# krzkro4122/vit-gan

Hardware: AMD Instinct MI355X
Metric: images/sec (G+D step) ViTGAN 32x32 patch4 dim384 (higher is better)
Workload: dtype bf16; 1 GPU; C2: CIFAR-10-shaped 3x32x32, patch 4 (65 tokens), E=384, 4 heads, 6 blocks ViT discriminator + SLN/SIREN generator (z=1024, 32 tokens, 4 blocks), full alternating G+D step, AdamW; fp8_attention=False, per_gpu_batch=256, global_batch=256, loss=ns, parallelism=dp1, hip_graph=True, compress_mapping_grad=False, fused_real_fake_pass=True, losses_finite=True

## Files before the change

include/vitgan_hip.h:

```cpp
#ifndef VITGAN_HIP_H
#define VITGAN_HIP_H

#include <stdint.h>

#ifdef __cplusplus
extern "C" {
#endif

#define VG_ABI_VERSION 9
int vg_abi_version(void);


int vg_linear_fwd(const void* A, const void* W, const float* bias, const void* res, void* C,
                  void* pre_bf16, float* pre_f32, int M, int N, int K, int act, float act_scale,
                  void* stream);
int vg_linear_gelu_fwd(const void* A, const void* W, const float* bias, void* C, void* dcode, int M, int N, int K,
                       void* stream);
int vg_linear_dgrad(const void* dY, const void* W, void* dX, int M, int N, int K, int mul_mode,
                    const void* Z, const float* Zf, float act_scale, void* stream);
#define VG_WGRAD_MAX_SPLITS 64
long long vg_linear_wgrad_slab_floats(int N, int K, int splits);
int vg_linear_wgrad(const void* dY, const void* X, float* dW, float* slab_ws, long long slab_floats, int M,
                    int N, int K, int splits, int accumulate, void* stream);
int vg_linear_wgrad_group(int n, const void* const* dY, const void* const* X, const int* N, const int* K, const long long* off,
// ... 49 lines not shown

long long vg_encoder_post_attention_image_elems(void);
int vg_encoder_post_attention_pack(const void* Wo, const void* W1, const void* W2, void* img, void* stream);
int vg_encoder_post_attention_fwd(const void* ao, const void* x, const void* img, const float* bo, const float* b1, const float* b2,
                                  const float* gamma2, const float* beta2, const float* gamma, const float* beta, void* xmid, void* xn2,
                                  float* mean2, float* rstd2, void* a1, void* dcode, void* Y, void* Yn, float* mean, float* rstd, int M,
                                  float eps, float drop_p, unsigned long long seed, int site_attn, int site_mlp,
                                  const unsigned* step_dev, void* stream);

int vg_linear_sln_fwd(const void* A, const void* Wp, const float* bias, const void* res, const float* resf, int res_period,
                      void* Y, void* Yn, float* mean, float* rstd, const void* wmod, const float* lw, const float* lb,
                      const float* gs, const float* bs, int M, int K, float eps, float drop_p, unsigned long long seed,
                      int site, const unsigned* step_dev, void* stream);
int vg_linear_dgrad_sln_bwd(const void* dY, const void* WpT, const void* h, int h_bcast_rows, const void* wmod,
                            const float* mean, const float* rstd, const float* lw, const float* lb, const float* gs,
                            const float* bs, const void* gres, void* dh, void* dhm, float* dw_acc, int dw_accumulate,
                            float* part, int M, int K, float drop_p, unsigned long long seed, int site,
                            const unsigned* step_dev, void* stream);

int vg_colsum_f32(const float* part, int rows, int width, float* d0, int n0, float* d1, int n1,
                  float* d2, int n2, float* d3, int n3, int accumulate, void* stream);

int vg_colsum_bf16_parts(int R);
int vg_colsum_bf16(const void* X, long long ld, int R, int N, float* part_ws, float* dst, int accumulate,
                   void* stream);

int vg_dropout_apply(const void* x, void* y, long long n, float p, unsigned long long seed, int site,
                     const unsigned* step_dev, void* stream);

int vg_attention_fwd(const void* qkv, void* out, float* lse, int B, int H, int S, int HE,
                     float scale, void* stream);
int vg_attention_bwd(const void* qkv, const void* out, const void* d_out, const float* lse,
                     void* d_qkv, int B, int H, int S, int HE, float scale, void* stream);
int vg_attention_cls_fwd(const void* qkv, void* out_cls, float* lse_cls, int B, int H, int S, int HE, float scale, void* stream);
int vg_attention_cls_bwd(const void* qkv, const void* out_cls, const void* d_out_cls, const float* lse_cls, void* d_qkv, int B, int H,
                         int S, int HE, float scale, void* stream);

int vg_attention_fp8_fwd(const void* qkv, void* out, float* lse, int B, int H, int S, int HE,
                         float scale, void* stream);
int vg_attention_fp8_bwd(const void* qkv, const void* out, const void* d_out, const float* lse,
                         void* d_qkv, int B, int H, int S, int HE, float scale, void* stream);

int vg_attention_l2_fwd(const void* qkv, void* out, float* lse, int B, int H, int S, int HE,
                        float scale, void* stream);
int vg_attention_l2_bwd(const void* qkv, const void* out, const void* d_out, const float* lse,
                        void* d_qkv, int B, int H, int S, int HE, float scale, void* stream);

int vg_unfold_tokens_fwd(const void* img, int img_is_bf16, void* tokens, int B, int C, int IH, int P,
                         int overlap, void* stream);
int vg_unfold_tokens_bwd(const void* d_tokens, void* d_img, int B, int C, int IH, int P, int overlap,
                         void* stream);

int vg_act_fwd(const void* h, void* y, long long n, int act, void* stream);
int vg_act_bwd(const void* dy, const void* h, void* dh, long long n, int act, void* stream);
int vg_act_bwd_bwd(const void* u, const void* dy, const void* h, void* d_dy, void* d_h, long long n, int act,
                   void* stream);
int vg_layernorm_bwd_bwd_parts(int R);
int vg_layernorm_bwd_bwd(const void* u, const void* dy, const void* x, const float* mean, const float* rstd,
                         const float* gamma, void* d_dy, void* d_x, float* part, int R, int E, void* stream);
int vg_attention_bwd_bwd(const void* qkv, const void* d_out, const float* lse, const void* u_qkv, void* d_d_out,
                         void* d_qkv2, int B, int H, int S, int HE, float scale, void* stream);

int vg_zero_tick(float* g, long long n, int* step_dev, void* stream);
int vg_step_inputs(const float* real, void* imgs_bf16, long long n_img, float* z, long long n_z,
                   unsigned long long seed, const int* step_dev, void* stream);

// ... 199 lines not shown
```

vit-gan_amd/_lib.py:

```python
from __future__ import annotations

import ctypes as C
import os
import subprocess
from typing import Optional

_HERE = os.path.dirname(os.path.abspath(__file__))
LIB_PATH = os.environ.get("VITGAN_HIP_LIB", os.path.join(_HERE, "libvitgan_hip.so"))
CSRC = os.path.join(_HERE, "csrc")

c_void_p, c_int, c_float, c_ll = C.c_void_p, C.c_int, C.c_float, C.c_longlong
ABI_VERSION = 9


class VgVitDims(C.Structure):
    _fields_ = [(n, c_int) for n in ("C", "IH", "P", "E", "H", "L", "R", "Kc")]


class VgVitLayout(C.Structure):
    _fields_ = [(n, c_ll) for n in (
        "conv_w", "conv_b", "pos", "cls", "layer0", "layer_stride", "wqkv", "wo", "w1", "w2",
        "ln1_w", "ln1_b", "bqkv", "bo", "ln2_w", "ln2_b", "b1", "b2", "layer_weights",
        "lnf_w", "lnf_b", "hw1", "hb1", "hw2", "hb2", "total")]

# ... 53 lines not shown
    "vg_linear_wgrad_slab_floats": (c_ll, [c_int, c_int, c_int]),
    "vg_linear_wgrad": (c_int, [P, P, P, P, c_ll, c_int, c_int, c_int, c_int, c_int, P]),
    "vg_linear_wgrad_group": (c_int, [c_int, P, P, P, P, P, c_int, c_int, P, c_ll, P, c_ll, c_int, P]),
    "vg_layernorm_fwd": (c_int, [P, c_ll, P, P, P, c_ll, P, P, c_int, c_int, c_float, P]),
    "vg_layernorm_bwd_parts": (c_int, [c_int]),
    "vg_layernorm_bwd": (c_int, [P, P, P, P, P, P, P, P, c_int, c_int, P]),
    "vg_sln_fwd": (c_int, [P, c_int, P, P, P, P, P, P, P, P, c_int, c_int, c_float, P]),
    "vg_sln_bwd": (c_int, [P, P, c_int, P, P, P, P, P, P, P, P, P, P, c_int, P, c_int, c_int, P]),
    "vg_row_pack_elems": (c_ll, [c_int]),
    "vg_row_pack_weight": (c_int, [P, c_int, c_int, c_int, P, P]),
    "vg_row_parts": (c_int, [c_int]),
    "vg_linear_ln_fwd": (c_int, [P, P, P, P, P, P, P, P, P, P, c_int, c_int, c_float, c_float, C.c_ulonglong, c_int, P, P]),
    "vg_linear_dgrad_ln_bwd": (c_int, [P, P, P, P, P, P, P, P, P, P, c_int, c_int, c_float, C.c_ulonglong, c_int, P, P]),
    "vg_row_pack_elems_e": (c_ll, [c_int, c_int]),
    "vg_row_pack_weight_e": (c_int, [c_int, P, c_int, c_int, c_int, P, P]),
    "vg_linear_ln_fwd_e": (c_int, [c_int, P, P, P, P, P, P, P, P, P, P, c_int, c_int, c_float, c_float, C.c_ulonglong, c_int, P, P]),
    "vg_linear_dgrad_ln_bwd_e": (c_int, [c_int, P, P, P, P, P, P, P, P, P, P, c_int, c_int, c_float, C.c_ulonglong, c_int, P, P]),
    "vg_linear_sln_fwd_e": (c_int, [c_int, P, P, P, P, P, c_int, P, P, P, P, P, P, P, P, P, c_int, c_int, c_float, c_float, C.c_ulonglong, c_int, P, P]),
    "vg_linear_dgrad_sln_bwd_e": (c_int, [c_int, P, P, P, c_int, P, P, P, P, P, P, P, P, P, P, P, c_int, P, c_int, c_int, c_float, C.c_ulonglong, c_int, P, P]),
    "vg_encoder_mlp_image_elems": (c_ll, []),
    "vg_encoder_mlp_pack": (c_int, [P, P, P, P]),
    "vg_encoder_mlp_fwd": (c_int, [P, P, P, P, P, P, P, P, P, P, P, P, P, c_int, c_float, c_float, C.c_ulonglong, c_int, P, P]),
    "vg_encoder_post_attention_image_elems": (c_ll, []),
    "vg_encoder_post_attention_pack": (c_int, [P, P, P, P, P]),
    "vg_encoder_post_attention_fwd": (c_int, [P] * 20 + [c_int, c_float, c_float, C.c_ulonglong, c_int, c_int, P, P]),
    "vg_linear_sln_fwd": (c_int, [P, P, P, P, P, c_int, P, P, P, P, P, P, P, P, P, c_int, c_int, c_float, c_float, C.c_ulonglong, c_int, P, P]),
    "vg_linear_dgrad_sln_bwd": (c_int, [P, P, P, c_int, P, P, P, P, P, P, P, P, P, P, P, c_int, P, c_int, c_int, c_float, C.c_ulonglong, c_int, P, P]),
    "vg_colsum_f32": (c_int, [P, c_int, c_int, P, c_int, P, c_int, P, c_int, P, c_int, c_int, P]),
    "vg_colsum_bf16_parts": (c_int, [c_int]),
    "vg_colsum_bf16": (c_int, [P, c_ll, c_int, c_int, P, P, c_int, P]),
    "vg_dropout_apply": (c_int, [P, P, c_ll, c_float, C.c_ulonglong, c_int, P, P]),
    "vg_attention_fwd": (c_int, [P, P, P, c_int, c_int, c_int, c_int, c_float, P]),
    "vg_attention_bwd": (c_int, [P, P, P, P, P, c_int, c_int, c_int, c_int, c_float, P]),
    "vg_attention_cls_fwd": (c_int, [P, P, P, c_int, c_int, c_int, c_int, c_float, P]),
    "vg_attention_cls_bwd": (c_int, [P, P, P, P, P, c_int, c_int, c_int, c_int, c_float, P]),
    "vg_unfold_tokens_fwd": (c_int, [P, c_int, P, c_int, c_int, c_int, c_int, c_int, P]),
    "vg_unfold_tokens_bwd": (c_int, [P, P, c_int, c_int, c_int, c_int, c_int, P]),
    "vg_attention_fp8_fwd": (c_int, [P, P, P, c_int, c_int, c_int, c_int, c_float, P]),
    "vg_attention_fp8_bwd": (c_int, [P, P, P, P, P, c_int, c_int, c_int, c_int, c_float, P]),
    "vg_attention_l2_fwd": (c_int, [P, P, P, c_int, c_int, c_int, c_int, c_float, P]),
    "vg_attention_l2_bwd": (c_int, [P, P, P, P, P, c_int, c_int, c_int, c_int, c_float, P]),
    "vg_act_fwd": (c_int, [P, P, c_ll, c_int, P]),
    "vg_act_bwd": (c_int, [P, P, P, c_ll, c_int, P]),
    "vg_act_bwd_bwd": (c_int, [P, P, P, P, P, c_ll, c_int, P]),
    "vg_layernorm_bwd_bwd_parts": (c_int, [c_int]),
    "vg_layernorm_bwd_bwd": (c_int, [P, P, P, P, P, P, P, P, P, c_int, c_int, P]),
    "vg_attention_bwd_bwd": (c_int, [P, P, P, P, P, P, c_int, c_int, c_int, c_int, c_float, P]),
    "vg_zero_tick": (c_int, [P, c_ll, P, P]),
    "vg_step_inputs": (c_int, [P, P, c_ll, P, c_ll, C.c_ulonglong, P, P]),
    "vg_diffaug_fwd": (c_int, [P, P, P, c_int, c_int, c_int, c_int, C.c_ulonglong, c_int, P, P]),
    "vg_diffaug_bwd": (c_int, [P, P, c_int, c_int, c_int, c_int, c_int, C.c_ulonglong, c_int, P, P]),
    "vg_diffaug_p_fwd": (c_int, [P, P, P, c_int, c_int, c_int, c_int, C.c_ulonglong, c_int, P, P, P]),
    "vg_diffaug_p_bwd": (c_int, [P, P, c_int, c_int, c_int, c_int, c_int, C.c_ulonglong, c_int, P, P, P]),
    "vg_ada_update": (c_int, [P, c_int, P, c_float, c_float, c_int, P, P]),
    "vg_gan_loss": (c_int, [P, P, P, c_int, c_int, c_int, c_float, P]),
    "vg_gan_loss_pair": (c_int, [P, P, P, c_int, c_int, c_int, c_int, c_int, c_float, P]),
    "vg_bcr_loss": (c_int, [P, P, P, P, P, c_int, c_int, c_int, c_float, c_float, c_int, c_int, c_float, P]),
    "vg_adamw_step": (c_int, [P, P, P, P, P, c_ll, c_float, c_float, c_float, c_float, c_float, c_int, P, c_float, P]),
    "vg_adamw_ema_step": (c_int, [P, P, P, P, P, P, c_ll, c_float, c_float, c_float, c_float, c_float, c_int, P, c_float, c_float, c_int, P]),
    "vg_adamw_step_dlr": (c_int, [P, P, P, P, P, c_ll, P, c_float, c_float, c_float, c_float, c_int, P, c_float, P]),
    "vg_adamw_ema_step_dlr": (c_int, [P, P, P, P, P, P, c_ll, P, c_float, c_float, c_float, c_float, c_int, P, c_float, c_float, c_int, P]),
    "vg_lr_schedule": (c_int, [C.POINTER(VgLrSched), C.POINTER(VgLrSched), P, P, P, P]),
    "vg_ema_update": (c_int, [P, P, c_ll, c_float, c_int, c_int, P, P]),
    "vg_diversity_loss": (c_int, [P, P, P, P, c_int, c_int, c_float, P]),
    "vg_grad_clip": (c_int, [P, c_ll, c_float, c_float, P, P]),
    "vg_cast_f32_bf16": (c_int, [P, P, c_ll, P]),
# ... 94 lines not shown
```

vit-gan_amd/csrc/attention.hip:

```cpp
#include "vg_attn.h"
#include "vg_kernels.h"

typedef long fp8x8;
__device__ __forceinline__ fp8x8 to_fp8(float a0, float a1, float a2, float a3, float a4, float a5, float a6, float a7) {
  int lo = 0, hi = 0;
  lo = __builtin_amdgcn_cvt_pk_fp8_f32(a0, a1, lo, false);
  lo = __builtin_amdgcn_cvt_pk_fp8_f32(a2, a3, lo, true);
  hi = __builtin_amdgcn_cvt_pk_fp8_f32(a4, a5, hi, false);
  hi = __builtin_amdgcn_cvt_pk_fp8_f32(a6, a7, hi, true);
  return (fp8x8)(((unsigned long)(unsigned)hi << 32) | (unsigned long)(unsigned)lo);
}
__device__ __forceinline__ fp8x8 to_fp8(bf16x8 v) {
  return to_fp8(vg_bf2f(v[0]), vg_bf2f(v[1]), vg_bf2f(v[2]), vg_bf2f(v[3]), vg_bf2f(v[4]), vg_bf2f(v[5]), vg_bf2f(v[6]), vg_bf2f(v[7]));
}
__device__ __forceinline__ fp8x8 pack_pair_fp8(f32x4 a, f32x4 b, float mul) {
  return to_fp8(a[0] * mul, a[1] * mul, a[2] * mul, a[3] * mul, b[0] * mul, b[1] * mul, b[2] * mul, b[3] * mul);
}
__device__ __forceinline__ f32x4 vg_mfma_fp8(fp8x8 a, fp8x8 b, f32x4 c) { return __builtin_amdgcn_mfma_f32_16x16x32_fp8_fp8(a, b, c, 0, 0, 0); }
template <bool FP8>
__device__ __forceinline__ f32x4 score_mfma(bf16x8 a, bf16x8 b, f32x4 c) {
  if constexpr (FP8) return vg_mfma_fp8(to_fp8(a), to_fp8(b), c);
  else return vg_mfma(a, b, c);
}
#define VG_P_FP8_SCALE 256.0f
// ... 383 lines not shown
      f32x4 s = zero, dp = zero;
#pragma unroll
      for (int ks = 0; ks < KS; ++ks) {
        s = score_mfma<FP8>(lfrag_row<HE>(s0, 16 * qt, ks, lane), kf[ks], s);
        dp = vg_mfma(lfrag_row<HE>(s1, 16 * qt, ks, lane), vf[ks], dp);
      }
      const f32x4 lq4 = *(const f32x4*)(ll + 16 * qt + 4 * g);
      const f32x4 dl4 = *(const f32x4*)(dl + 16 * qt + 4 * g);
#pragma unroll
      for (int r = 0; r < 4; ++r) {
        const int q = 16 * qt + 4 * g + r;
        const float p = ((q < S) && (key < S)) ? __expf(s[r] * scale - lq4[r]) : 0.f;
        pr[qt][r] = p;
        ds[qt][r] = p * (dp[r] - dl4[r]) * scale;
      }
    }
    bf16x8 pf[KP], dsf[KP];
#pragma unroll
    for (int u = 0; u < KP; ++u) {
      const int hi = (2 * u + 1 < NT) ? 2 * u + 1 : 0;
      pf[u] = pack_pair(pr[2 * u], (2 * u + 1 < NT) ? pr[hi] : zero);
      dsf[u] = pack_pair(ds[2 * u], (2 * u + 1 < NT) ? ds[hi] : zero);
    }
    bf16* rowp = dqb + (size_t)(key < S ? key : 0) * ld;
#pragma unroll
    for (int pp = 0; pp < DT / 2; ++pp) {
      f32x4 dv[2] = {zero, zero}, dk[2] = {zero, zero};
#pragma unroll
      for (int u = 0; u < KP; ++u) {
#pragma unroll
        for (int t = 0; t < 2; ++t) {
          dv[t] = vg_mfma(lfrag_tr<HE>(s1, u, 32 * pp + 16 * t, lane), pf[u], dv[t]);
          dk[t] = vg_mfma(lfrag_tr<HE>(s0, u, 32 * pp + 16 * t, lane), dsf[u], dk[t]);
        }
      }
      store_tiles<2>(rowp + E + 32 * pp, dk, 1.0f, g, key < S);
      store_tiles<2>(rowp + 2 * E + 32 * pp, dv, 1.0f, g, key < S);
    }
  }
}

template <int HE>
__global__ __launch_bounds__(320, 2) void vg_attn_bwd_bwd2_kernel(const bf16* __restrict__ qkv, const bf16* __restrict__ d_o,
                                                                  const float* __restrict__ lse, const bf16* __restrict__ uqkv,
                                                                  bf16* __restrict__ d_do, bf16* __restrict__ d_qkv, int B, int S, int H,
                                                                  float scale, const void* __restrict__ zeros) {
  constexpr int NT = 5, KS = HE / 32, DT = HE / 16, KP = 3, RP = 96;
  constexpr int IMG = RP * HE * 2;
  __shared__ __attribute__((aligned(16))) unsigned char sm[4 * IMG + 4 * RP * 4];
  unsigned char* i0 = sm;
  unsigned char* i1 = sm + IMG;
  unsigned char* i2 = sm + 2 * IMG;
  unsigned char* i3 = sm + 3 * IMG;
  float* dl = (float*)(sm + 4 * IMG);
  float* gm = dl + RP;
  float* pl = gm + RP;
  float* ll = pl + RP;
  int b, h;
  if (!attn_block(B, H, b, h)) return;
  const int tid = threadIdx.x, lane = tid & 63, wv = tid >> 6;
  const int g = lane >> 4, li = lane & 15;
  const int E = H * HE;
  const size_t ld = 3 * (size_t)E;
  const bf16* qb = qkv + (size_t)b * S * ld + h * HE;
  const bf16* kb = qb + E;
  const bf16* vb = qb + 2 * E;
// ... 160 lines not shown
    for (int pp = 0; pp < DT / 2; ++pp) {
      f32x4 dk[2] = {zero, zero}, dv[2] = {zero, zero};
#pragma unroll
      for (int u = 0; u < KP; ++u)
#pragma unroll
        for (int t = 0; t < 2; ++t) {
          const int d0 = 32 * pp + 16 * t;
          dk[t] = vg_mfma(lfrag_tr<HE>(i2, u, d0, lane), dsf[u], dk[t]);
          dk[t] = vg_mfma(lfrag_tr<HE>(i0, u, d0, lane), sgf[u], dk[t]);
          dv[t] = vg_mfma(lfrag_tr<HE>(i1, u, d0, lane), hf[u], dv[t]);
        }
      store_tiles<2>(rowp + E + 32 * pp, dk, scale, g, key < S);
      store_tiles<2>(rowp + 2 * E + 32 * pp, dv, 1.0f, g, key < S);
    }
  }
}

__device__ __attribute__((aligned(16))) unsigned int vg_attn_zero_page[4] = {0u, 0u, 0u, 0u};
static const void* attn_zeros() {
  static void* zp = nullptr;
  if (!zp && hipGetSymbolAddress(&zp, HIP_SYMBOL(vg_attn_zero_page)) != hipSuccess) zp = nullptr;
  return zp;
}

template <int HE, int NT, int MODE>
static int launch_fwd(const bf16* qkv, bf16* o, float* lse, int B, int H, int S, float scale, hipStream_t st) {
  const void* z = attn_zeros();
  if (!z) return -5;
  hipLaunchKernelGGL((vg_attn_fwd_kernel<HE, NT, MODE == 1, MODE == 2>), dim3(attn_grid(B, H)), dim3(64 * NT), 0, st, qkv, o, lse, B, S, H, scale, z);
  return (int)hipGetLastError();
}
template <int HE, int NT, int MODE>
static int launch_bwd(const bf16* qkv, const bf16* o, const bf16* d_o, const float* lse, bf16* dqkv, int B, int H,
                      int S, float scale, hipStream_t st) {
  const void* z = attn_zeros();
  if (!z) return -5;
#ifndef VG_ATTN_BWD_4IMG
  if constexpr (MODE != 1 && NT == 5) {
    hipLaunchKernelGGL((vg_attn_bwd2_kernel<HE, NT, MODE == 2>), dim3(attn_grid(B, H)), dim3(64 * NT), 0, st, qkv, o, d_o, lse, dqkv, B, S, H, scale, z);
    return (int)hipGetLastError();
  }
#endif
  hipLaunchKernelGGL((vg_attn_bwd_kernel<HE, NT, MODE == 1, MODE == 2>), dim3(attn_grid(B, H)), dim3(64 * NT), 0, st, qkv, o, d_o, lse, dqkv, B, S, H, scale, z);
  return (int)hipGetLastError();
}

#define VG_ATTN_BY_NT(FN, HE_, MODE_, ...) return small ? FN<HE_, 2, MODE_>(__VA_ARGS__) : FN<HE_, 5, MODE_>(__VA_ARGS__)
#define VG_ATTN_BY_MODE(FN, HE_, ...)                                  \
  do {                                                                 \
    if (mode == 0) { VG_ATTN_BY_NT(FN, HE_, 0, __VA_ARGS__); }         \
    if (mode == 1) { VG_ATTN_BY_NT(FN, HE_, 1, __VA_ARGS__); }         \
    VG_ATTN_BY_NT(FN, HE_, 2, __VA_ARGS__);                            \
  } while (0)
#define VG_ATTN_DISPATCH(FN, ...)                                      \
  do {                                                                 \
    if (S < 1 || S > 80 || B < 1 || H < 1) return -2;                  \
    if (mode < 0 || mode > 2) return -4;                               \
    const bool small = (S <= 32);                                      \
    if (HE == 96) VG_ATTN_BY_MODE(FN, 96, __VA_ARGS__);                \
    if (HE == 64) VG_ATTN_BY_MODE(FN, 64, __VA_ARGS__);                \
    if (HE == 32) VG_ATTN_BY_MODE(FN, 32, __VA_ARGS__);                \
    return -3;                                                         \
  } while (0)
int vg_attn_fwd_launch(const bf16* qkv, bf16* o, float* lse, int B, int H, int S, int HE, float scale, int mode, hipStream_t st) {
  if (mode == 0 && S > VG_SHORT_MAX_S && S <= VG_ATTN_LONG_MAX_S) return vg_attn_long_fwd_launch(qkv, o, lse, B, H, S, HE, scale, st);
  VG_ATTN_DISPATCH(launch_fwd, qkv, o, lse, B, H, S, scale, st);
}
int vg_attn_bwd_launch(const bf16* qkv, const bf16* o, const bf16* d_o, const float* lse, bf16* dqkv, int B, int H,
                       int S, int HE, float scale, int mode, hipStream_t st) {
  if (mode == 0 && S > VG_SHORT_MAX_S && S <= VG_ATTN_LONG_MAX_S) return vg_attn_long_bwd_launch(qkv, o, d_o, lse, dqkv, B, H, S, HE, scale, st);
  VG_ATTN_DISPATCH(launch_bwd, qkv, o, d_o, lse, dqkv, B, H, S, scale, st);
}

template <int HE, int KMAX>
__global__ __launch_bounds__(64) void vg_attn_cls_fwd_kernel(const bf16* __restrict__ qkv, bf16* __restrict__ o_cls, float* __restrict__ lse_cls,
                                                             int B, int S, int H, float scale) {
  constexpr int CPR = HE / 8, RPI = 64 / CPR;
  __shared__ float q0l[HE];
  constexpr int NR = KMAX / 64;
  __shared__ float part[KMAX * CPR];
  __shared__ float pl[KMAX];
  int b, h;
  if (!attn_block(B, H, b, h)) return;
  const int lane = threadIdx.x;
  const int rr = lane / CPR, c = lane - rr * CPR;
  const bool act = rr < RPI;
  const int E = H * HE;
  const size_t ld = 3 * (size_t)E;
  const bf16* qb = qkv + (size_t)b * S * ld + h * HE;
  const bf16* kb = qb + E;
  const bf16* vb = qb + 2 * E;
  for (int d = lane; d < HE; d += 64) q0l[d] = vg_bf2f(qb[d]);
  __syncthreads();
  float qc[8];
#pragma unroll
  for (int t = 0; t < 8; ++t) qc[t] = q0l[8 * (act ? c : 0) + t];
  for (int r0 = 0; r0 < S; r0 += RPI) {
    const int r = r0 + rr;
    if (act && r < S) {
      const bf16x8 k8 = *(const bf16x8*)(kb + (size_t)r * ld + 8 * c);
      float a = 0.f;
#pragma unroll
      for (int t = 0; t < 8; ++t) a = fmaf(qc[t], vg_bf2f(k8[t]), a);
      part[r * CPR + c] = a;
// ... 174 lines not shown
```

vit-gan_amd/csrc/capi.hip:

```cpp
#include "../../include/vitgan_hip.h"
#include "vg_kernels.h"
#include "vg_row.h"
#include "vg_chain.h"
#include "vg_spectral.h"
#include <algorithm>
#include <cstring>
#include <vector>

extern "C" int vg_abi_version(void) { return VG_ABI_VERSION; }

extern "C" int vg_linear_fwd(const void* A, const void* W, const float* bias, const void* res, void* C, void* pre_bf16,
                             float* pre_f32, int M, int N, int K, int act, float act_scale, void* stream) {
  if (!A || !W || (!C && !pre_bf16 && !pre_f32)) return -1;
  if (act < 0 || act > 3) return -4;
  VgGemmProb p = vg_gemm_prob();
  p.A = (const bf16*)A; p.lda = K; p.B = (const bf16*)W; p.ldb = K; p.M = M; p.N = N; p.K = K;
  p.C = (bf16*)C; p.ldc = N; p.bias = bias; p.res = (const bf16*)res; p.ldr = N; p.C2 = (bf16*)pre_bf16; p.ldc2 = N;
  if (pre_f32) { p.pre_f32 = 1; p.Cf = pre_f32; p.ldcf = N; }
  p.act = act; p.act_scale = act_scale;
  return vg_gemm_launch(&p, 1, VG_NT, (hipStream_t)stream);
}
extern "C" int vg_linear_gelu_fwd(const void* A, const void* W, const float* bias, void* C, void* dcode, int M, int N, int K, void* stream) {
  if (!A || !W || !C || !dcode) return -1;
  VgGemmProb p = vg_gemm_prob();
// ... 235 lines not shown
  ra.N = E;
  ra.A = (const bf16*)dY; ra.lda = K; ra.Wp = (const bf16*)WpT; ra.M = M; ra.K = K; ra.x = (const bf16*)x; ra.mean = mean; ra.rstd = rstd;
  ra.gamma = gamma; ra.gres = (const bf16*)gres; ra.dx = (bf16*)dx; ra.dxm = (bf16*)dxm; ra.part = part;
  if (dxm) row_drop(ra, drop_p, seed, site, step_dev);
  if (dxm && !ra.drop_thresh) { ra.drop_thresh = 0; ra.drop_scale = 1.f; }
  const int r = vg_gemm_row_launch(ra, VG_ROW_LNBWD, (hipStream_t)stream);
  return r > 0 ? 0 : (r < 0 ? -r : -3);
}
extern "C" int vg_linear_dgrad_ln_bwd(const void* dY, const void* WpT, const void* x, const float* mean, const float* rstd,
                                      const float* gamma, const void* gres, void* dx, void* dxm, float* part, int M, int K,
                                      float drop_p, unsigned long long seed, int site, const unsigned* step_dev, void* stream) {
  return vg_linear_dgrad_ln_bwd_e(VG_ROW_N, dY, WpT, x, mean, rstd, gamma, gres, dx, dxm, part, M, K, drop_p, seed, site, step_dev, stream);
}
extern "C" int vg_attention_fwd(const void* qkv, void* out, float* lse, int B, int H, int S, int HE, float scale, void* stream) {
  if (!qkv || !out || !lse) return -1;
  return vg_attn_fwd_launch((const bf16*)qkv, (bf16*)out, lse, B, H, S, HE, scale, 0, (hipStream_t)stream);
}
extern "C" int vg_attention_cls_fwd(const void* qkv, void* out_cls, float* lse_cls, int B, int H, int S, int HE, float scale, void* stream) {
  if (!qkv || !out_cls || !lse_cls) return -1;
  return vg_attn_cls_fwd_launch((const bf16*)qkv, (bf16*)out_cls, lse_cls, B, H, S, HE, scale, (hipStream_t)stream);
}
extern "C" int vg_attention_cls_bwd(const void* qkv, const void* out_cls, const void* d_out_cls, const float* lse_cls, void* d_qkv, int B, int H,
                                    int S, int HE, float scale, void* stream) {
  if (!qkv || !out_cls || !d_out_cls || !lse_cls || !d_qkv) return -1;
  return vg_attn_cls_bwd_launch((const bf16*)qkv, (const bf16*)out_cls, (const bf16*)d_out_cls, lse_cls, (bf16*)d_qkv, B, H, S, HE, scale,
                                (hipStream_t)stream);
}
extern "C" int vg_attention_bwd(const void* qkv, const void* out, const void* d_out, const float* lse, void* d_qkv, int B, int H,
                                int S, int HE, float scale, void* stream) {
  if (!qkv || !out || !d_out || !lse || !d_qkv) return -1;
  return vg_attn_bwd_launch((const bf16*)qkv, (const bf16*)out, (const bf16*)d_out, lse, (bf16*)d_qkv, B, H, S, HE, scale, 0,
                            (hipStream_t)stream);
}
extern "C" int vg_attention_fp8_fwd(const void* qkv, void* out, float* lse, int B, int H, int S, int HE, float scale, void* stream) {
  if (!qkv || !out || !lse) return -1;
  return vg_attn_fwd_launch((const bf16*)qkv, (bf16*)out, lse, B, H, S, HE, scale, 2, (hipStream_t)stream);
}
extern "C" int vg_attention_fp8_bwd(const void* qkv, const void* out, const void* d_out, const float* lse, void* d_qkv, int B, int H,
                                    int S, int HE, float scale, void* stream) {
  if (!qkv || !out || !d_out || !lse || !d_qkv) return -1;
  return vg_attn_bwd_launch((const bf16*)qkv, (const bf16*)out, (const bf16*)d_out, lse, (bf16*)d_qkv, B, H, S, HE, scale, 2,
                            (hipStream_t)stream);
}
extern "C" int vg_attention_l2_fwd(const void* qkv, void* out, float* lse, int B, int H, int S, int HE, float scale, void* stream) {
  if (!qkv || !out || !lse) return -1;
  return vg_attn_fwd_launch((const bf16*)qkv, (bf16*)out, lse, B, H, S, HE, scale, 1, (hipStream_t)stream);
}
extern "C" int vg_attention_l2_bwd(const void* qkv, const void* out, const void* d_out, const float* lse, void* d_qkv, int B, int H,
                                   int S, int HE, float scale, void* stream) {
  if (!qkv || !out || !d_out || !lse || !d_qkv) return -1;
  return vg_attn_bwd_launch((const bf16*)qkv, (const bf16*)out, (const bf16*)d_out, lse, (bf16*)d_qkv, B, H, S, HE, scale, 1,
                            (hipStream_t)stream);
}
extern "C" int vg_unfold_tokens_fwd(const void* img, int img_is_bf16, void* tokens, int B, int C, int IH, int P, int overlap, void* stream) {
  if (!img || !tokens || B < 1 || C < 1) return -1;
  return vg_unfold_tokens_launch(img, img_is_bf16, (bf16*)tokens, B, C, IH, P, overlap, (hipStream_t)stream);
}
extern "C" int vg_unfold_tokens_bwd(const void* d_tokens, void* d_img, int B, int C, int IH, int P, int overlap, void* stream) {
  if (!d_tokens || !d_img || B < 1 || C < 1) return -1;
  return vg_unfold_tokens_bwd_launch((const bf16*)d_tokens, (bf16*)d_img, B, C, IH, P, overlap, (hipStream_t)stream);
}
extern "C" int vg_act_fwd(const void* h, void* y, long long n, int act, void* stream) {
  if (!h || !y || n < 1) return -1;
  return vg_act2_launch((const bf16*)h, nullptr, nullptr, (bf16*)y, nullptr, n, act, 0, (hipStream_t)stream);
}
extern "C" int vg_act_bwd(const void* dy, const void* h, void* dh, long long n, int act, void* stream) {
// ... 188 lines not shown
```

vit-gan_amd/csrc/vg_attn.h:

```cpp
#pragma once
#include "vg_common.h"

template <int HE>
__device__ __forceinline__ int swz_chunk(int r, int c) {
  if (HE == 64) return (((c >> 1) ^ ((r >> 1) & 3)) << 1) | ((c & 1) ^ ((r >> 3) & 1));
  const int x = (r >> 2) & 3;
  return (c & ~3) | ((c & 3) ^ (((x & 1) << 1) | (x >> 1)));
}
template <int HE>
__device__ __forceinline__ int lds_off(int r, int d) {
  return r * (HE * 2) + (swz_chunk<HE>(r, d >> 3) << 4) + ((d & 7) << 1);
}

typedef const __attribute__((address_space(1))) void* gptr_t;
typedef __attribute__((address_space(3))) void* lptr_t;
template <int HE, int NW>
__device__ __forceinline__ void dma_head(unsigned char* img, const bf16* __restrict__ src, size_t ld, int S, int rows_alloc,
                                         const void* zeros, int wave, int lane) {
  constexpr int CPR = HE / 8;
  const int pieces = rows_alloc * CPR / 64;
  for (int pc = wave; pc < pieces; pc += NW) {
    const int ci = 64 * pc + lane;
    const int r = ci / CPR, cp = ci - r * CPR;
    const int c = swz_chunk<HE>(r, cp);
// ... 10 lines not shown
    bf16x8 w;
#pragma unroll
    for (int r = 0; r < 4; ++r) {
      const auto sw = __builtin_amdgcn_permlane16_swap(__float_as_uint(te[r] * mul), __float_as_uint(to[r] * mul), false, false);
      w[r] = vg_f2bf(__uint_as_float(sw[0]));
      w[r + 4] = vg_f2bf(__uint_as_float(sw[1]));
    }
    if (ok) *(bf16x8*)(rowp + 32 * pr + ((g & 1) << 4) + ((g & 2) << 2)) = w;
  }
}

__device__ __forceinline__ bf16x8 gfrag(const bf16* __restrict__ src, size_t ld, int r0, int ks, int S, int lane) {
  const int row = r0 + (lane & 15), d = 32 * ks + 8 * (lane >> 4);
  bf16x8 z = {0, 0, 0, 0, 0, 0, 0, 0};
  if (row < S) z = *(const bf16x8*)(src + (size_t)row * ld + d);
  return z;
}
template <int HE>
__device__ __forceinline__ bf16x8 lfrag_row(const unsigned char* lds, int r0, int ks, int lane) {
  return *(const bf16x8*)(lds + lds_off<HE>(r0 + (lane & 15), 32 * ks + 8 * (lane >> 4)));
}
template <int HE>
__device__ __forceinline__ bf16x8 lfrag_tr(const unsigned char* lds, int u, int d0, int lane) {
  const int g = lane >> 4, li = lane & 15, q = li >> 2, p = li & 3;
  typedef bf16x4 __attribute__((address_space(3))) * lds4;
  const int r = 32 * u + 4 * g + q;
  bf16x4 lo = __builtin_amdgcn_ds_read_tr16_b64_v4bf16((lds4)(lds + lds_off<HE>(r, d0 + 4 * p)));
  bf16x4 hi = __builtin_amdgcn_ds_read_tr16_b64_v4bf16((lds4)(lds + lds_off<HE>(r + 16, d0 + 4 * p)));
  bf16x8 o;
  o[0] = lo[0]; o[1] = lo[1]; o[2] = lo[2]; o[3] = lo[3];
  o[4] = hi[0]; o[5] = hi[1]; o[6] = hi[2]; o[7] = hi[3];
  return o;
}
__device__ __forceinline__ bf16x8 pack_pair(f32x4 a, f32x4 b) {
  bf16x8 o;
#pragma unroll
  for (int j = 0; j < 4; ++j) { o[j] = vg_f2bf(a[j]); o[j + 4] = vg_f2bf(b[j]); }
  return o;
}
__device__ __forceinline__ float group_sum(float v) {
  v += __shfl_xor(v, 16, 64);
  v += __shfl_xor(v, 32, 64);
  return v;
}
__device__ __forceinline__ float group_max(float v) {
  v = fmaxf(v, __shfl_xor(v, 16, 64));
  v = fmaxf(v, __shfl_xor(v, 32, 64));
  return v;
}

__device__ __forceinline__ bool attn_block(int B, int H, int& b, int& h) {
#ifdef VG_ATTN_LINEAR_MAP
  b = blockIdx.x / H; h = blockIdx.x - b * H;
#else
  const int x = blockIdx.x & 7, i = blockIdx.x >> 3;
  b = (i / H) * 8 + x; h = i % H;
#endif
  return b < B;
}
static inline int attn_grid(int B, int H) { return ((B + 7) / 8) * 8 * H; }
```

vit-gan_amd/csrc/vg_kernels.h:

```cpp
#pragma once
#include "vg_common.h"
#include "vg_gemm.h"

int vg_attn_fwd_launch(const bf16* qkv, bf16* o, float* lse, int B, int H, int S, int HE, float scale, int mode, hipStream_t st);
int vg_attn_bwd_launch(const bf16* qkv, const bf16* o, const bf16* d_o, const float* lse, bf16* dqkv, int B, int H,
                       int S, int HE, float scale, int mode, hipStream_t st);
#define VG_SHORT_MAX_S 80
#define VG_ATTN_LONG_MAX_S 256
int vg_attn_long_fwd_launch(const bf16* qkv, bf16* o, float* lse, int B, int H, int S, int HE, float scale, hipStream_t st);
int vg_attn_long_bwd_launch(const bf16* qkv, const bf16* o, const bf16* d_o, const float* lse, bf16* dqkv, int B, int H, int S, int HE,
                            float scale, hipStream_t st);

int vg_ln_fwd_launch(const bf16* x, long long xs, const float* gamma, const float* beta, bf16* y, long long ys,
                     float* mean, float* rstd, int R, int E, float eps, hipStream_t st);
int vg_sln_fwd_launch(const bf16* h, int h_bcast_rows, const bf16* wmod, const float* lw, const float* lb,
                      const float* gs, const float* bs, bf16* y, float* mean, float* rstd, int R, int E, float eps,
                      hipStream_t st);
int vg_ln_bwd_nparts(int R);
int vg_ln_bwd_launch(const bf16* dy, const bf16* x, const float* mean, const float* rstd, const float* gamma,
                     const bf16* gres, bf16* dx, float* part, int R, int E, bf16* dxm, unsigned dthr, unsigned dkey,
                     float dscale, const unsigned* dstep, hipStream_t st, int x_row_step = 1, int drop_row_mul = 1);
int vg_sln_bwd_launch(const bf16* dy, const bf16* h, int h_bcast_rows, const bf16* wmod, const float* mean,
                      const float* rstd, const float* lw, const float* lb, const float* gs, const float* bs,
                      const bf16* gres, bf16* dh, float* dw_acc, int dw_accumulate, float* part, int R, int E,
                      bf16* dhm, unsigned dthr, unsigned dkey, float dscale, const unsigned* dstep, hipStream_t st);
int vg_colsum_f32_launch(const float* part, int rows, int width, float* d0, int n0, float* d1, int n1, float* d2, int n2,
                         float* d3, int n3, int accumulate, hipStream_t st);
#include "vg_fold.h"
int vg_colsum_f32_multi_launch(const VgFoldJobs& jobs, hipStream_t st);
int vg_colsum_bf16_nparts(int R);
int vg_colsum_bf16_part_launch(const bf16* X, long long ld, int R, int N, float* part, hipStream_t st);
int vg_colsum_bf16_launch(const bf16* X, long long ld, int R, int N, float* part, float* dst, int accumulate,
                          hipStream_t st);

int vg_patchify_launch(const void* img, int img_is_bf16, bf16* A, int B, int C, int IH, int P, hipStream_t st);
int vg_unpatchify_launch(const bf16* dA, bf16* dimg, int B, int C, int IH, int P, hipStream_t st);
int vg_embed_fused_ok(int C, int IH, int P, int E);
int vg_embed_fwd_launch(const void* img, int img_is_bf16, const bf16* W, const float* bias, const float* pos, const float* cls, const float* gamma,
                        const float* beta, bf16* Apatch, bf16* X, bf16* Xn, float* mean, float* rstd, int B, int C, int IH, float eps, unsigned dthr,
// ... 103 lines not shown
```

Measured before the change: 49020 images/sec.

## Add compact-LDS three-image attention backward kernel and form selector

Adds a new attention backward kernel that stages K, V and dO into compactly packed LDS images sized by the actual sequence length and reuses the V slot for Q after the dQ pass. Padded rows are redirected to a shared zero area rather than stored. When the compact layout fits, the default dispatch now chooses this kernel over the previous bwd2 kernel, aiming to cut LDS footprint and wasted DMA for short sequences (65 tokens, head dim 96). A form-selection API is exposed for testing; the rewritten kernel risks correctness or scheduling regressions from inline-asm m0 handling.

```diff
diff --git a/include/vitgan_hip.h b/include/vitgan_hip.h
--- a/include/vitgan_hip.h
+++ b/include/vitgan_hip.h
@@ -105,6 +105,8 @@
                      float scale, void* stream);
 int vg_attention_bwd(const void* qkv, const void* out, const void* d_out, const float* lse,
                      void* d_qkv, int B, int H, int S, int HE, float scale, void* stream);
+int vg_attention_bwd_form(const void* qkv, const void* out, const void* d_out, const float* lse,
+                          void* d_qkv, int B, int H, int S, int HE, float scale, int fp8, int form, void* stream);
 int vg_attention_cls_fwd(const void* qkv, void* out_cls, float* lse_cls, int B, int H, int S, int HE, float scale, void* stream);
 int vg_attention_cls_bwd(const void* qkv, const void* out_cls, const void* d_out_cls, const float* lse_cls, void* d_qkv, int B, int H,
                          int S, int HE, float scale, void* stream);
diff --git a/vit-gan_amd/_lib.py b/vit-gan_amd/_lib.py
--- a/vit-gan_amd/_lib.py
+++ b/vit-gan_amd/_lib.py
@@ -109,6 +109,7 @@
     "vg_dropout_apply": (c_int, [P, P, c_ll, c_float, C.c_ulonglong, c_int, P, P]),
     "vg_attention_fwd": (c_int, [P, P, P, c_int, c_int, c_int, c_int, c_float, P]),
     "vg_attention_bwd": (c_int, [P, P, P, P, P, c_int, c_int, c_int, c_int, c_float, P]),
+    "vg_attention_bwd_form": (c_int, [P, P, P, P, P, c_int, c_int, c_int, c_int, c_float, c_int, c_int, P]),
     "vg_attention_cls_fwd": (c_int, [P, P, P, c_int, c_int, c_int, c_int, c_float, P]),
     "vg_attention_cls_bwd": (c_int, [P, P, P, P, P, c_int, c_int, c_int, c_int, c_float, P]),
     "vg_unfold_tokens_fwd": (c_int, [P, c_int, P, c_int, c_int, c_int, c_int, c_int, P]),
diff --git a/vit-gan_amd/csrc/attention.hip b/vit-gan_amd/csrc/attention.hip
--- a/vit-gan_amd/csrc/attention.hip
+++ b/vit-gan_amd/csrc/attention.hip
@@ -439,6 +439,158 @@
         for (int t = 0; t < 2; ++t) {
           dv[t] = vg_mfma(lfrag_tr<HE>(s1, u, 32 * pp + 16 * t, lane), pf[u], dv[t]);
           dk[t] = vg_mfma(lfrag_tr<HE>(s0, u, 32 * pp + 16 * t, lane), dsf[u], dk[t]);
+        }
+      }
+      store_tiles<2>(rowp + E + 32 * pp, dk, 1.0f, g, key < S);
+      store_tiles<2>(rowp + 2 * E + 32 * pp, dv, 1.0f, g, key < S);
+    }
+  }
+}
+
+template <int HE>
+struct attn_compact { static constexpr int MAXP = HE == 96 ? 13 : HE == 64 ? 10 : 5; };
+template <int HE, int NT, bool FP8>
+__global__ __launch_bounds__(64 * NT, VG_ATTN_BWD2_WPE) void vg_attn_bwd3_kernel(const bf16* __restrict__ qkv, const bf16* __restrict__ o,
+                                                                  const bf16* __restrict__ d_o, const float* __restrict__ lse,
+                                                                  bf16* __restrict__ dqkv, int B, int S, int H, float scale,
+                                                                  const void* __restrict__ zeros) {
+  constexpr int KS = HE / 32, DT = HE / 16, KP = (NT + 1) / 2, RQ = 16 * NT;
+  constexpr int IMG = attn_compact<HE>::MAXP * 1024;
+  constexpr int I0 = 0, I1 = IMG, I2 = 2 * IMG, ZERO = 3 * IMG;
+  __shared__ __attribute__((aligned(256))) unsigned char sm[3 * IMG + VG_ATTN_ZERO_AREA + 2 * RQ * 4];
+  float* dl = (float*)(sm + ZERO + VG_ATTN_ZERO_AREA);
+  float* ll = dl + RQ;
+  int b, h;
+  if (!attn_block(B, H, b, h)) return;
+  const int tid = threadIdx.x, lane = tid & 63, wv = tid >> 6;
+  const int g = lane >> 4, li = lane & 15;
+  const int E = H * HE;
+  const size_t ld = 3 * (size_t)E;
+  const bf16* qb = qkv + (size_t)b * S * ld + h * HE;
+  const bf16* kb = qb + E;
+  const bf16* vb = qb + 2 * E;
+  const bf16* ob = o + (size_t)b * S * E + h * HE;
+  const bf16* dob = d_o + (size_t)b * S * E + h * HE;
+  const float* lb = lse + ((size_t)b * H + h) * S;
+  bf16* dqb = dqkv + (size_t)b * S * ld + h * HE;
+  const f32x4 zero = {0.f, 0.f, 0.f, 0.f};
+  const int pieces = compact_pieces<HE>(S);
+  cfrag_t<HE> cf(S, ZERO, lane);
+
+  dma_head_compact<HE, NT>(sm + I0, kb, ld, S, pieces, zeros, wv, lane);
+  dma_head_compact<HE, NT>(sm + I1, vb, ld, S, pieces, zeros, (wv + 2) % NT, lane);
+  dma_head_compact<HE, NT>(sm + I2, dob, (size_t)E, S, pieces, zeros, (wv + 4) % NT, lane);
+  bf16x8 qf[KS], dof[KS];
+  float delta;
+  {
+    bf16x8 of[KS];
+#pragma unroll
+    for (int ks = 0; ks < KS; ++ks) {
+      of[ks] = gfrag(ob, (size_t)E, 16 * wv, ks, S, lane);
+      qf[ks] = gfrag(qb, ld, 16 * wv, ks, S, lane);
+    }
+    for (int i = tid; i < RQ; i += 64 * NT) ll[i] = (i < S) ? lb[i] : 0.f;
+    if (tid < VG_ATTN_ZERO_AREA / 16) *(f32x4*)(sm + ZERO + 16 * tid) = zero;
+    asm volatile("s_waitcnt vmcnt(0)" ::: "memory");
+    __syncthreads();
+    float dpart = 0.f;
+#pragma unroll
+    for (int ks = 0; ks < KS; ++ks) {
+      dof[ks] = cf.row(sm, I2, wv, ks);
+#pragma unroll
+      for (int j = 0; j < 8; ++j) dpart += vg_bf2f(dof[ks][j]) * vg_bf2f(of[ks][j]);
+    }
+    delta = group_sum(dpart);
+    if (g == 0) dl[16 * wv + li] = delta;
+  }
+
+  bf16x8 vf[KS];
+  {
+    const int q = 16 * wv + li;
+    const float lse_q = ll[q];
+    f32x4 ds[NT];
+#pragma unroll
+    for (int kt = 0; kt < NT; ++kt) {
+      f32x4 st = zero, dpt = zero;
+#pragma unroll
+      for (int ks = 0; ks < KS; ++ks) {
+        st = score_mfma<FP8>(cf.row(sm, I0, kt, ks), qf[ks], st);
+        dpt = vg_mfma(cf.row(sm, I1, kt, ks), dof[ks], dpt);
+      }
+#pragma unroll
+      for (int r = 0; r < 4; ++r) {
+        const int key = 16 * kt + 4 * g + r;
+        const float p = (key < S && q < S) ? __expf(st[r] * scale - lse_q) : 0.f;
+        ds[kt][r] = p * (dpt[r] - delta) * scale;
+      }
+    }
+#pragma unroll
+    for (int ks = 0; ks < KS; ++ks) vf[ks] = cf.row(sm, I1, wv, ks);
+    bf16x8 dsf[KP];
+#pragma unroll
+    for (int u = 0; u < KP; ++u) {
+      dsf[u] = pack_pair(ds[2 * u], (2 * u + 1 < NT) ? ds[(2 * u + 1 < NT) ? 2 * u + 1 : 0] : zero);
+      asm volatile("" : "+v"(dsf[u]));
+    }
+    __syncthreads();
+    cf.renew();
+    dma_head_compact_unordered<HE, NT>(sm + I1, qb, ld, S, pieces, zeros, wv, lane);
+    bf16* rowq = dqb + (size_t)(q < S ? q : 0) * ld;
+#pragma unroll
+    for (int pp = 0; pp < DT / 2; ++pp) {
+      f32x4 dq[2] = {zero, zero};
+#pragma unroll
+      for (int u = 0; u < KP; ++u) {
+        dq[0] = vg_mfma(cf.tr(sm, I0, u, 2 * pp), dsf[u], dq[0]);
+        dq[1] = vg_mfma(cf.tr(sm, I0, u, 2 * pp + 1), dsf[u], dq[1]);
+      }
+      store_tiles<2>(rowq + 32 * pp, dq, 1.0f, g, q < S);
+    }
+  }
+  asm volatile("s_waitcnt vmcnt(0)" ::: "memory");
+  __syncthreads();
+  {
+    const int key = 16 * wv + li;
+    cf.renew();
+    bf16x8 kf[KS];
+#pragma unroll
+    for (int ks = 0; ks < KS; ++ks) kf[ks] = cf.row(sm, I0, wv, ks);
+    f32x4 pr[NT], ds[NT];
+#pragma unroll
+    for (int qt = 0; qt < NT; ++qt) {
+      f32x4 s = zero, dp = zero;
+#pragma unroll
+      for (int ks = 0; ks < KS; ++ks) {
+        s = score_mfma<FP8>(cf.row(sm, I1, qt, ks), kf[ks], s);
+        dp = vg_mfma(cf.row(sm, I2, qt, ks), vf[ks], dp);
+      }
+      const f32x4 lq4 = *(const f32x4*)(ll + 16 * qt + 4 * g);
+      const f32x4 dl4 = *(const f32x4*)(dl + 16 * qt + 4 * g);
+#pragma unroll
+      for (int r = 0; r < 4; ++r) {
+        const int q = 16 * qt + 4 * g + r;
+        const float p = ((q < S) && (key < S)) ? __expf(s[r] * scale - lq4[r]) : 0.f;
+        pr[qt][r] = p;
+        ds[qt][r] = p * (dp[r] - dl4[r]) * scale;
+      }
+    }
+    bf16x8 pf[KP], dsf[KP];
+#pragma unroll
+    for (int u = 0; u < KP; ++u) {
+      const int hi = (2 * u + 1 < NT) ? 2 * u + 1 : 0;
+      pf[u] = pack_pair(pr[2 * u], (2 * u + 1 < NT) ? pr[hi] : zero);
+      dsf[u] = pack_pair(ds[2 * u], (2 * u + 1 < NT) ? ds[hi] : zero);
+    }
+    bf16* rowp = dqb + (size_t)(key < S ? key : 0) * ld;
+#pragma unroll
+    for (int pp = 0; pp < DT / 2; ++pp) {
+      f32x4 dv[2] = {zero, zero}, dk[2] = {zero, zero};
+#pragma unroll
+      for (int u = 0; u < KP; ++u) {
+#pragma unroll
+        for (int t = 0; t < 2; ++t) {
+          dv[t] = vg_mfma(cf.tr(sm, I2, u, 2 * pp + t), pf[u], dv[t]);
+          dk[t] = vg_mfma(cf.tr(sm, I1, u, 2 * pp + t), dsf[u], dk[t]);
         }
       }
       store_tiles<2>(rowp + E + 32 * pp, dk, 1.0f, g, key < S);
@@ -665,15 +817,24 @@
 }
 template <int HE, int NT, int MODE>
 static int launch_bwd(const bf16* qkv, const bf16* o, const bf16* d_o, const float* lse, bf16* dqkv, int B, int H,
-                      int S, float scale, hipStream_t st) {
+                      int S, float scale, int form, hipStream_t st) {
   const void* z = attn_zeros();
   if (!z) return -5;
 #ifndef VG_ATTN_BWD_4IMG
   if constexpr (MODE != 1 && NT == 5) {
-    hipLaunchKernelGGL((vg_attn_bwd2_kernel<HE, NT, MODE == 2>), dim3(attn_grid(B, H)), dim3(64 * NT), 0, st, qkv, o, d_o, lse, dqkv, B, S, H, scale, z);
+    const bool fits = compact_pieces<HE>(S) <= attn_compact<HE>::MAXP;
+    if (form == 2 && !fits) return -2;
+#ifdef VG_ATTN_BWD_2IMG
+    if (form == 0) form = 1;
+#endif
+    if (form == 2 || (form == 0 && fits))
+      hipLaunchKernelGGL((vg_attn_bwd3_kernel<HE, NT, MODE == 2>), dim3(attn_grid(B, H)), dim3(64 * NT), 0, st, qkv, o, d_o, lse, dqkv, B, S, H, scale, z);
+    else
+      hipLaunchKernelGGL((vg_attn_bwd2_kernel<HE, NT, MODE == 2>), dim3(attn_grid(B, H)), dim3(64 * NT), 0, st, qkv, o, d_o, lse, dqkv, B, S, H, scale, z);
     return (int)hipGetLastError();
   }
 #endif
+  if (form != 0) return -2;
   hipLaunchKernelGGL((vg_attn_bwd_kernel<HE, NT, MODE == 1, MODE == 2>), dim3(attn_grid(B, H)), dim3(64 * NT), 0, st, qkv, o, d_o, lse, dqkv, B, S, H, scale, z);
   return (int)hipGetLastError();
 }
@@ -702,7 +863,13 @@
 int vg_attn_bwd_launch(const bf16* qkv, const bf16* o, const bf16* d_o, const float* lse, bf16* dqkv, int B, int H,
                        int S, int HE, float scale, int mode, hipStream_t st) {
   if (mode == 0 && S > VG_SHORT_MAX_S && S <= VG_ATTN_LONG_MAX_S) return vg_attn_long_bwd_launch(qkv, o, d_o, lse, dqkv, B, H, S, HE, scale, st);
-  VG_ATTN_DISPATCH(launch_bwd, qkv, o, d_o, lse, dqkv, B, H, S, scale, st);
+  VG_ATTN_DISPATCH(launch_bwd, qkv, o, d_o, lse, dqkv, B, H, S, scale, 0, st);
+}
+int vg_attn_bwd_form_launch(const bf16* qkv, const bf16* o, const bf16* d_o, const float* lse, bf16* dqkv, int B, int H,
+                            int S, int HE, float scale, int mode, int form, hipStream_t st) {
+  if (form == 0) return vg_attn_bwd_launch(qkv, o, d_o, lse, dqkv, B, H, S, HE, scale, mode, st);
+  if (form < 0 || form > 2) return -4;
+  VG_ATTN_DISPATCH(launch_bwd, qkv, o, d_o, lse, dqkv, B, H, S, scale, form, st);
 }
 
 template <int HE, int KMAX>
diff --git a/vit-gan_amd/csrc/capi.hip b/vit-gan_amd/csrc/capi.hip
--- a/vit-gan_amd/csrc/capi.hip
+++ b/vit-gan_amd/csrc/capi.hip
@@ -291,6 +291,12 @@
   return vg_attn_bwd_launch((const bf16*)qkv, (const bf16*)out, (const bf16*)d_out, lse, (bf16*)d_qkv, B, H, S, HE, scale, 0,
                             (hipStream_t)stream);
 }
+extern "C" int vg_attention_bwd_form(const void* qkv, const void* out, const void* d_out, const float* lse, void* d_qkv, int B, int H,
+                                     int S, int HE, float scale, int fp8, int form, void* stream) {
+  if (!qkv || !out || !d_out || !lse || !d_qkv) return -1;
+  return vg_attn_bwd_form_launch((const bf16*)qkv, (const bf16*)out, (const bf16*)d_out, lse, (bf16*)d_qkv, B, H, S, HE, scale, fp8 ? 2 : 0,
+                                 form, (hipStream_t)stream);
+}
 extern "C" int vg_attention_fp8_fwd(const void* qkv, void* out, float* lse, int B, int H, int S, int HE, float scale, void* stream) {
   if (!qkv || !out || !lse) return -1;
   return vg_attn_fwd_launch((const bf16*)qkv, (bf16*)out, lse, B, H, S, HE, scale, 2, (hipStream_t)stream);
diff --git a/vit-gan_amd/csrc/vg_attn.h b/vit-gan_amd/csrc/vg_attn.h
--- a/vit-gan_amd/csrc/vg_attn.h
+++ b/vit-gan_amd/csrc/vg_attn.h
@@ -66,6 +66,77 @@
   o[4] = hi[0]; o[5] = hi[1]; o[6] = hi[2]; o[7] = hi[3];
   return o;
 }
+template <int HE>
+__host__ __device__ constexpr int compact_pieces(int S) { return (S * (HE / 8) + 63) / 64; }
+#define VG_ATTN_ZERO_AREA 384
+template <int HE, int NW>
+__device__ __forceinline__ void dma_head_compact(unsigned char* img, const bf16* __restrict__ src, size_t ld, int S, int pieces,
+                                                 const void* zeros, int wave, int lane) {
+  constexpr int CPR = HE / 8;
+  for (int pc = wave; pc < pieces; pc += NW) {
+    const int ci = 64 * pc + lane;
+    const int r = ci / CPR, cp = ci - r * CPR;
+    const int c = swz_chunk<HE>(r, cp);
+    const void* p = (r < S) ? (const void*)(src + (size_t)r * ld + 8 * c) : zeros;
+    __builtin_amdgcn_global_load_lds((gptr_t)p, (lptr_t)(img + 1024 * pc), 16, 0, 0);
+  }
+}
+template <int HE, int NW>
+__device__ __forceinline__ void dma_head_compact_unordered(unsigned char* img, const bf16* __restrict__ src, size_t ld, int S, int pieces,
+                                                           const void* zeros, int wave, int lane) {
+  constexpr int CPR = HE / 8;
+  const unsigned dst0 = (unsigned)(unsigned long)(lptr_t)img;
+  const int w0 = __builtin_amdgcn_readfirstlane(wave);
+  for (int pc = w0; pc < pieces; pc += NW) {
+    const int ci = 64 * pc + lane;
+    const int r = ci / CPR, cp = ci - r * CPR;
+    const int c = swz_chunk<HE>(r, cp);
+    const void* p = (r < S) ? (const void*)(src + (size_t)r * ld + 8 * c) : zeros;
+    const unsigned dst = __builtin_amdgcn_readfirstlane(dst0 + 1024u * (unsigned)pc);
+    unsigned keep;
+    asm volatile("s_mov_b32 %0, m0\n\ts_mov_b32 m0, %2\n\ts_nop 0\n\tglobal_load_lds_dwordx4 %1, off\n\ts_mov_b32 m0, %0"
+                 : "=&s"(keep) : "v"(p), "s"(dst) : "memory");
+  }
+}
+template <int HE>
+struct cfrag_t {
+  static constexpr int NR = HE == 64 ? HE / 32 : 1, NTB = HE == 64 ? HE / 16 : 2;
+  int S, zero, rrow, trow;
+  int rb[NR], tb[NTB];
+  __device__ __forceinline__ cfrag_t(int S_, int zero_, int lane) : S(S_), zero(zero_) {
+    const int g = lane >> 4, li = lane & 15;
+    rrow = li;
+    trow = 4 * g + (li >> 2);
+#pragma unroll
+    for (int i = 0; i < NR; ++i) rb[i] = lds_off<HE>(rrow, 32 * i + 8 * g);
+#pragma unroll
+    for (int i = 0; i < NTB; ++i) tb[i] = lds_off<HE>(trow, 16 * i + 4 * (li & 3));
+  }
+  __device__ __forceinline__ void renew() {
+#pragma unroll
+    for (int i = 0; i < NR; ++i) asm volatile("" : "+v"(rb[i]));
+#pragma unroll
+    for (int i = 0; i < NTB; ++i) asm volatile("" : "+v"(tb[i]));
+  }
+  __device__ __forceinline__ bf16x8 row(const unsigned char* lds, int img, int t, int ks) const {
+    const int i = HE == 64 ? ks : 0, imm = HE == 64 ? 0 : 64 * ks;
+    const int a = (16 * t + rrow < S) ? img + 32 * HE * t + rb[i] : zero + (rb[i] & 255);
+    return *(const bf16x8*)(lds + a + imm);
+  }
+  __device__ __forceinline__ bf16x8 tr(const unsigned char* lds, int img, int u, int dt) const {
+    typedef bf16x4 __attribute__((address_space(3))) * lds4;
+    const int i = HE == 64 ? dt : (dt & 1), imm = HE == 64 ? 0 : 64 * (dt >> 1);
+    const int z = zero + (tb[i] & 255);
+    const int a0 = (32 * u + trow < S) ? img + 32 * HE * (2 * u) + tb[i] : z;
+    const int a1 = (32 * u + 16 + trow < S) ? img + 32 * HE * (2 * u + 1) + tb[i] : z;
+    bf16x4 lo = __builtin_amdgcn_ds_read_tr16_b64_v4bf16((lds4)(lds + a0 + imm));
+    bf16x4 hi = __builtin_amdgcn_ds_read_tr16_b64_v4bf16((lds4)(lds + a1 + imm));
+    bf16x8 o;
+    o[0] = lo[0]; o[1] = lo[1]; o[2] = lo[2]; o[3] = lo[3];
+    o[4] = hi[0]; o[5] = hi[1]; o[6] = hi[2]; o[7] = hi[3];
+    return o;
+  }
+};
 __device__ __forceinline__ bf16x8 pack_pair(f32x4 a, f32x4 b) {
   bf16x8 o;
 #pragma unroll
diff --git a/vit-gan_amd/csrc/vg_kernels.h b/vit-gan_amd/csrc/vg_kernels.h
--- a/vit-gan_amd/csrc/vg_kernels.h
+++ b/vit-gan_amd/csrc/vg_kernels.h
@@ -5,6 +5,8 @@
 int vg_attn_fwd_launch(const bf16* qkv, bf16* o, float* lse, int B, int H, int S, int HE, float scale, int mode, hipStream_t st);
 int vg_attn_bwd_launch(const bf16* qkv, const bf16* o, const bf16* d_o, const float* lse, bf16* dqkv, int B, int H,
                        int S, int HE, float scale, int mode, hipStream_t st);
+int vg_attn_bwd_form_launch(const bf16* qkv, const bf16* o, const bf16* d_o, const float* lse, bf16* dqkv, int B, int H,
+                            int S, int HE, float scale, int mode, int form, hipStream_t st);
 #define VG_SHORT_MAX_S 80
 #define VG_ATTN_LONG_MAX_S 256
 int vg_attn_long_fwd_launch(const bf16* qkv, bf16* o, float* lse, int B, int H, int S, int HE, float scale, hipStream_t st);
```

Result: no change. 49150 images/sec (median of 6 runs) (+0.3%).
